# minyoungg/pix2latent

Hardware: AMD Instinct MI355X
Metric: candidate-latent evals/sec (fwd+loss+bwd), BigGAN-256 pop=18 (higher is better)
Workload: dtype f32 (fp32 tensors everywhere; convolutions >= 32x32 and the self-attention multiply on the 16-bit MFMA pipe with fp32-grade operand splits and fp32 accumulate: the 16x16 Winograd, direct and sub-pixel 3x3 kernels and the 1x1 kernels (4x4 layers included) on power-of-two scaled operands in 2 fp16 pie

## Files before the change

pix2latent_amd/csrc/p2l_h2r.hip:

```cpp
#include "p2l_conv_k.h"

#include <atomic>
#include <type_traits>

using namespace p2lconv;

namespace {

#ifndef P2L_H2R_ABL
#define P2L_H2R_ABL 0
#endif

__device__ __forceinline__ int h2c(int c, int row) { return c ^ ((row >> 2) & 3) ^ (((row >> 1) & 1) << 1); }

constexpr int HP = 24, HH = 10, HW = 18;
constexpr int ROWS = HH * HP;
constexpr int PLANE = ROWS * 64 + 32;
constexpr int BUF = 4 * PLANE;
constexpr int EP = 68;
constexpr int DUMP_FLOATS = 4 * 32 * EP;
constexpr int ETAB_FLOATS = 4 * 16 * 12;
constexpr int PTAB_FLOATS = 16 * 8;
constexpr size_t LDS_BYTES = 2 * (size_t)BUF + (DUMP_FLOATS + 32 + ETAB_FLOATS + PTAB_FLOATS) * sizeof(float);

template <int PRO, int EPI>
__global__ __launch_bounds__(256, 1) void conv_h2r_kernel(const ConvK k, const int n_tiles) {
  constexpr bool FAST = EPI != 0, MASK = EPI == 2, POOL = EPI == 3;
  extern __shared__ __attribute__((aligned(16))) float smem[];
  char* As = reinterpret_cast<char*>(smem);
  float* dump = smem + 2 * BUF / 4;
  float* red = dump + DUMP_FLOATS;
  float* etab = red + 32;
  float* ptab = etab + ETAB_FLOATS;

  const int tid = threadIdx.x;
  const int lane = tid & 63, wave = tid >> 6;
  const int l31 = lane & 31, lhi = lane >> 5;
  const int mh = wave >> 1, nt = wave & 1;

  h16x8 bh[36], bm[36];
  {
    const char* wb = reinterpret_cast<const char*>(k.w) + l31 * 64;
    const int oh = h2c(lhi, l31) * 16, om = h2c(2 + lhi, l31) * 16;
#pragma unroll
    for (int s = 0; s < 36; ++s) {
      const int c = s / 9, tap = s - c * 9;
      const char* slab = wb + (size_t)(((c * 2 + nt) * 9 + tap) * 32) * 64;
      bh[s] = *reinterpret_cast<const h16x8*>(slab + oh);
      bm[s] = *reinterpret_cast<const h16x8*>(slab + om);
    }
  }

  const int G = gridDim.x;
  const int v = xcd_remap(blockIdx.x, G);
  const int t_begin = (int)(((long)v * n_tiles) / G), t_end = (int)(((long)(v + 1) * n_tiles) / G);
  const int tiles_per_image = k.tiles_x * k.tiles_y;

  const int cq = tid & 15, p0 = tid >> 4;
  const int goff0 = (-k.W + (p0 - 1)) * k.x_ld + cq * 4;
  const int lplane = (cq >> 2) * PLANE;
  const int loff0 = p0 * 64 + (cq & 1) * 8 + h2c((cq >> 1) & 1, p0) * 16;
  int e_line[2], e_hx[2], e_goff[2], e_loff[2];
#pragma unroll
  for (int e = 0; e < 2; ++e) {
    const int idx = tid + 256 * e;
    e_line[e] = idx < 320 ? (idx >> 5) : -1;
    e_hx[e] = 16 + ((idx >> 4) & 1);
    const int row = (idx >> 5) * HP + e_hx[e];
    e_goff[e] = (((idx >> 5) - 1) * k.W + (e_hx[e] - 1)) * k.x_ld + cq * 4;
    e_loff[e] = row * 64 + (cq & 1) * 8 + h2c((cq >> 1) & 1, row) * 16;
  }
  const int line_step = k.W * k.x_ld;

  int aoff[2][3];
#pragma unroll
  for (int ms = 0; ms < 2; ++ms) {
    const int i = (mh * 2 + ms) * 32 + l31;
    const int Q = i >> 2, s = i & 3;
    const int row0 = (2 * ((Q >> 3) & 3) + (s >> 1)) * HP + 2 * (Q & 7) + (s & 1);
#pragma unroll
    for (int dx = 0; dx < 3; ++dx) aoff[ms][dx] = (row0 + dx) * 64 + h2c(lhi, row0 + dx) * 16;
  }

  float sw, inv_w;
  h2_scales(__builtin_amdgcn_readfirstlane(k.w_tail[0]), sw, inv_w);

  auto image_scales = [&](int b, float& xs, float& os) {
    float a = 0.f, ms_ = 0.f, mt_ = 0.f;
    if (k.amax_in != nullptr) {
      for (int i = tid; i < k.amax_in_n; i += 256) a = fmaxf(a, k.amax_in[(size_t)b * k.amax_in_n + i]);
      if (PRO != P2L_PRO_NONE && !k.amax_in_applied) {
        const f32x4* ps = reinterpret_cast<const f32x4*>(k.pro_s + (size_t)b * k.pro_bstride);
        const f32x4* pt = reinterpret_cast<const f32x4*>(k.pro_t + (size_t)b * k.pro_bstride);
        for (int c = tid; c < (k.Cin >> 2); c += 256) {
          const f32x4 s4 = ps[c], t4 = pt[c];
          ms_ = fmaxf(fmaxf(ms_, fmaxf(fabsf(s4.x), fabsf(s4.y))), fmaxf(fabsf(s4.z), fabsf(s4.w)));
          mt_ = fmaxf(fmaxf(mt_, fmaxf(fabsf(t4.x), fabsf(t4.y))), fmaxf(fabsf(t4.z), fabsf(t4.w)));
        }
      }
    } else if (tid < 64) {
      a = k.amax[b * 64 + tid];
    }
#pragma unroll
    for (int o = 1; o < 64; o <<= 1) {
      a = fmaxf(a, __shfl_xor(a, o, 64));
      if (PRO != P2L_PRO_NONE) { ms_ = fmaxf(ms_, __shfl_xor(ms_, o, 64)); mt_ = fmaxf(mt_, __shfl_xor(mt_, o, 64)); }
    }
    __syncthreads();
    if (lane == 0) { red[wave * 4] = a; red[wave * 4 + 1] = ms_; red[wave * 4 + 2] = mt_; }
    if (PRO != P2L_PRO_NONE && tid < 16) {
      *reinterpret_cast<f32x4*>(ptab + tid * 8) = *reinterpret_cast<const f32x4*>(k.pro_s + (size_t)b * k.pro_bstride + tid * 4);
      *reinterpret_cast<f32x4*>(ptab + tid * 8 + 4) = *reinterpret_cast<const f32x4*>(k.pro_t + (size_t)b * k.pro_bstride + tid * 4);
    }
    __syncthreads();
    a = fmaxf(fmaxf(red[0], red[4]), fmaxf(red[8], red[12]));
    ms_ = fmaxf(fmaxf(red[1], red[5]), fmaxf(red[9], red[13]));
    mt_ = fmaxf(fmaxf(red[2], red[6]), fmaxf(red[10], red[14]));
    if (PRO != P2L_PRO_NONE && k.amax_in != nullptr) a = (k.amax_in_applied ? a : ms_ * a + mt_) * 1.001f;
    float inv_x;
    h2_scales(__builtin_bit_cast(unsigned, a), xs, inv_x);
    os = inv_x * inv_w;
  };

  f32x4 xr[6];
  float st_xs = 1.f;
  char* st_dst = As;
  const float* st_base = k.x;
  bool st_top = false, st_bot = false, st_left = false, st_right = false;
  auto tile_geom = [&](int t, int& b, int& y0, int& x0, int& til) {
    b = t / tiles_per_image;
    til = t - b * tiles_per_image;
    const int ty = til / k.tiles_x;
    y0 = ty << 3; x0 = (til - ty * k.tiles_x) << 4;
  };
  auto item_ok = [&](int it) -> bool {
    if (it < 10) return !((st_top && it == 0) || (st_bot && it == 9) || (st_left && p0 == 0));
    const int e = it - 10;
    return e_line[e] >= 0 && !((st_top && e_line[e] == 0) || (st_bot && e_line[e] == 9) || (st_right && e_hx[e] == 17));
  };
  auto begin_tile = [&](int t, int buf, float xs) {
    int b, y0, x0, til;
    tile_geom(t, b, y0, x0, til);
    st_top = (y0 == 0); st_bot = (y0 + 8 == k.H); st_left = (x0 == 0); st_right = (x0 + 16 == k.W);
    st_xs = xs;
    st_dst = As + buf * BUF;
    st_base = k.x + (size_t)((b * k.H + y0) * k.W + x0) * k.x_ld;
  };
  auto issue = [&](auto half_c) {
    constexpr int half = decltype(half_c)::value;
#pragma unroll
    for (int j = 0; j < 6; ++j) {
      const int it = half * 6 + j;
      const int go = it < 10 ? goff0 + it * line_step : e_goff[it - 10];
      xr[j] = *reinterpret_cast<const f32x4*>(st_base + (item_ok(it) ? go : cq * 4));
    }
  };
  auto land = [&](int it) {
    if (it >= 10 && e_line[it - 10] < 0) return;
    f32x4 v4 = xr[it % 6];
    if (PRO != P2L_PRO_NONE) {
      const f32x4 s4 = *reinterpret_cast<const f32x4*>(ptab + cq * 8), t4 = *reinterpret_cast<const f32x4*>(ptab + cq * 8 + 4);
      v4 = v4 * s4 + t4;
      if (PRO == P2L_PRO_AFFINE_RELU) {
        v4.x = fmaxf(v4.x, 0.f); v4.y = fmaxf(v4.y, 0.f); v4.z = fmaxf(v4.z, 0.f); v4.w = fmaxf(v4.w, 0.f);
      }
    }
    v4 = v4 * (item_ok(it) ? st_xs : 0.f);
    const h16x4 h = __builtin_convertvector(v4, h16x4);
    const f32x4 w = __builtin_convertvector(h, f32x4);
    const h16x4 m = __builtin_convertvector(v4 - w, h16x4);
    const int lo = it < 10 ? ((loff0 + it * (HP * 64)) ^ ((it & 1) ? 32 : 0)) : e_loff[it - 10];
    *reinterpret_cast<h16x4*>(st_dst + lplane + lo) = h;
    *reinterpret_cast<h16x4*>(st_dst + lplane + (lo ^ 32)) = m;
  };
  using Half0 = std::integral_constant<int, 0>;
  using Half1 = std::integral_constant<int, 1>;

  const int e_c4 = lane & 15, e_n = e_c4 * 4;
  float* my_etab = etab + (wave * 16 + e_c4) * 12;
  f32x4 e_bias, e_ns, e_nt;
  if (FAST && lane < 16) {
    *reinterpret_cast<f32x4*>(my_etab) = k.bias ? ld4(k.bias, (unsigned)e_n) : f32x4{0.f, 0.f, 0.f, 0.f};
    *reinterpret_cast<f32x4*>(my_etab + 4) = f32x4{1.f, 1.f, 1.f, 1.f};
    *reinterpret_cast<f32x4*>(my_etab + 8) = f32x4{0.f, 0.f, 0.f, 0.f};
  }
  int e_tab_b = -1;
  const float e_lo = (k.act == P2L_ACT_RELU) ? 0.f : -__builtin_inff();
  int pb = 0, py0 = 0, px0 = 0, ptil = 0;
  float e_amax = 0.f, e_amaxp = 0.f;
  f32x4 ev, ep, em[4];
  unsigned e_pix0 = 0, e_ppix = 0;
  auto epi_tile = [&](int b, int y0_, int x0_, int til_) {
    pb = b; py0 = y0_; px0 = x0_; ptil = til_;
    e_amax = 0.f; e_amaxp = 0.f;
    if (k.amax_ps && b != e_tab_b) {
      if (lane < 16) {
        *reinterpret_cast<f32x4*>(my_etab + 4) = ld4(k.amax_ps, (unsigned)(b * k.amax_pbstride + e_n));
        *reinterpret_cast<f32x4*>(my_etab + 8) = ld4(k.amax_pt, (unsigned)(b * k.amax_pbstride + e_n));
      }
      e_tab_b = b;
    }
  };
  auto epi_addr = [&](int j) {
    const int Q = wave * 8 + j * 4 + (lane >> 4);
    const int oy0 = py0 + 2 * ((Q >> 3) & 3), ox0 = px0 + 2 * (Q & 7);
    e_pix0 = (unsigned)((pb * k.H + oy0) * k.W + ox0);
    e_ppix = (unsigned)((pb * (k.H >> 1) + (oy0 >> 1)) * (k.W >> 1) + (ox0 >> 1));
  };
  auto epi_mask = [&](int j) {
    epi_addr(j);
    if (MASK) {
#pragma unroll
      for (int s = 0; s < 4; ++s)
        em[s] = ld4(k.mask, (e_pix0 + (unsigned)((s >> 1) * k.W + (s & 1))) * (unsigned)k.mask_ld + (unsigned)e_n);
    }
  };
  auto epi_read = [&](int j, int s) {
    ev = *reinterpret_cast<const f32x4*>(dump + wave * 32 * EP + (4 * (j * 4 + (lane >> 4)) + s) * EP + e_c4 * 4);
    if (s == 0) {
      e_bias = *reinterpret_cast<const f32x4*>(my_etab);
      e_ns = *reinterpret_cast<const f32x4*>(my_etab + 4);
      e_nt = *reinterpret_cast<const f32x4*>(my_etab + 8);
    }
  };
  auto epi_px = [&](int s) {
    f32x4 t = ev + e_bias;
    t.x = fmaxf(t.x, e_lo); t.y = fmaxf(t.y, e_lo); t.z = fmaxf(t.z, e_lo); t.w = fmaxf(t.w, e_lo);
    if (MASK) {
      t.x = em[s].x > 0.f ? t.x : 0.f; t.y = em[s].y > 0.f ? t.y : 0.f;
      t.z = em[s].z > 0.f ? t.z : 0.f; t.w = em[s].w > 0.f ? t.w : 0.f;
    }
    st4(k.y, (e_pix0 + (unsigned)((s >> 1) * k.W + (s & 1))) * (unsigned)k.y_ld + (unsigned)e_n, t);
    e_amax = absmax4(e_amax, t * e_ns + e_nt);
    if (POOL) {
      if (s == 0) ep = t;
      else { ep.x = fmaxf(ep.x, t.x); ep.y = fmaxf(ep.y, t.y); ep.z = fmaxf(ep.z, t.z); ep.w = fmaxf(ep.w, t.w); }
    }
  };
  auto epi_pool = [&]() {
    if (POOL) {
      st4(k.yp, e_ppix * (unsigned)k.yp_ld + (unsigned)e_n, ep);
      e_amaxp = absmax4(e_amaxp, ep);
    }
  };
  auto epi_maxima = [&]() {
    if (k.amax_out != nullptr || k.amax_outp != nullptr) {
      float m = e_amax, mp = e_amaxp;
#pragma unroll
      for (int o = 1; o < 64; o <<= 1) { m = fmaxf(m, __shfl_xor(m, o, 64)); mp = fmaxf(mp, __shfl_xor(mp, o, 64)); }
      if (lane == 0) {
        const size_t slot = (size_t)pb * k.amax_out_n + (size_t)ptil * 4 + wave;
        if (k.amax_out != nullptr) k.amax_out[slot] = m;
        if (k.amax_outp != nullptr) k.amax_outp[slot] = mp;
      }
    }
  };
  auto epi_hook = [&](int s) {
    if (s == 0) epi_mask(0);
    if (s >= 5 && s < 9) epi_px(s - 5);
    if (s >= 4 && s < 8) epi_read(0, s - 4);
    if (s == 9) epi_pool();
    if (s == 16) epi_mask(1);
    if (s >= 21 && s < 25) epi_px(s - 21);
    if (s >= 20 && s < 24) epi_read(1, s - 20);
    if (s == 25) epi_pool();
  };

  if (t_begin >= t_end) return;

  int b_cur, y0, x0, til;
  tile_geom(t_begin, b_cur, y0, x0, til);
  float xs_cur, os_cur;
  image_scales(b_cur, xs_cur, os_cur);
  begin_tile(t_begin, 0, xs_cur);
  issue(Half0{});
#pragma unroll
  for (int it = 0; it < 6; ++it) land(it);
  issue(Half1{});
#pragma unroll
  for (int it = 6; it < 12; ++it) land(it);
  __syncthreads();

  auto run_tile = [&](int t, auto with_epi_c) {
    constexpr bool WITH_EPI = decltype(with_epi_c)::value;
    const int cur = (t - t_begin) & 1;
    tile_geom(t, b_cur, y0, x0, til);
    const int tn = (t + 1 < t_end) ? t + 1 : t;
    const int b_next = tn / tiles_per_image;
    float xs_next = xs_cur, os_next = os_cur;
    if (b_next != b_cur) image_scales(b_next, xs_next, os_next);
    begin_tile(tn, cur ^ 1, xs_next);
    if (!(P2L_H2R_ABL & 1)) issue(Half0{});

    const char* Ab = As + cur * BUF;
    f32x16 acc[2];
#pragma unroll
    for (int ms = 0; ms < 2; ++ms)
#pragma unroll
      for (int r = 0; r < 16; ++r) acc[ms][r] = 0.f;

    h16x8 af[2][2][2];
    auto lda = [&](int s, h16x8 (&a)[2][2]) {
      const int c = s / 9, tap = s - c * 9;
      const int dy = tap / 3, dx = tap - dy * 3;
#pragma unroll
      for (int ms = 0; ms < 2; ++ms) {
        const int oh = aoff[ms][dx] ^ ((dy & 1) ? 32 : 0);
        a[ms][0] = *reinterpret_cast<const h16x8*>(Ab + c * PLANE + dy * (HP * 64) + oh);
        a[ms][1] = *reinterpret_cast<const h16x8*>(Ab + c * PLANE + dy * (HP * 64) + (oh ^ 32));
      }
    };
    lda(0, af[0]);
#pragma unroll
    for (int s = 0; s < 36; ++s) {
      if (s + 1 < 36 && !(P2L_H2R_ABL & 16)) lda(s + 1, af[(s + 1) & 1]);
      __builtin_amdgcn_sched_barrier(0);
      const h16x8 (&a)[2][2] = af[s & 1];
      if (!(P2L_H2R_ABL & 2)) {
      acc[0] = __builtin_amdgcn_mfma_f32_32x32x16_f16(a[0][1], bh[s], acc[0], 0, 0, 0);
      acc[1] = __builtin_amdgcn_mfma_f32_32x32x16_f16(a[1][1], bh[s], acc[1], 0, 0, 0);
      acc[0] = __builtin_amdgcn_mfma_f32_32x32x16_f16(a[0][0], bm[s], acc[0], 0, 0, 0);
      acc[1] = __builtin_amdgcn_mfma_f32_32x32x16_f16(a[1][0], bm[s], acc[1], 0, 0, 0);
      acc[0] = __builtin_amdgcn_mfma_f32_32x32x16_f16(a[0][0], bh[s], acc[0], 0, 0, 0);
      acc[1] = __builtin_amdgcn_mfma_f32_32x32x16_f16(a[1][0], bh[s], acc[1], 0, 0, 0);
      } else { acc[0][s & 15] += (float)a[0][0][0] * (float)bh[s][0] + (float)a[1][1][1] * (float)bm[s][1]; }
      if (!(P2L_H2R_ABL & 1)) {
        if (s >= 10 && s < 16) land(s - 10);
        if (s == 15) issue(Half1{});
        if (s >= 28 && s < 34) land(s - 28 + 6);
      }
      if (WITH_EPI && !(P2L_H2R_ABL & 32)) epi_hook(s);
      __builtin_amdgcn_sched_barrier(0);
    }
    if (WITH_EPI) epi_maxima();

#pragma unroll
    for (int ms = 0; ms < 2; ++ms)
#pragma unroll
      for (int r = 0; r < 16; ++r) acc[ms][r] *= os_cur;
    __syncthreads();
    if (!(P2L_H2R_ABL & 8) || acc[0][0] == 12345.678f)
#pragma unroll
    for (int ms = 0; ms < 2; ++ms) {
      float* tb = dump + (mh * 2 + ms) * 32 * EP + nt * 32 + l31;
#pragma unroll
      for (int r = 0; r < 16; ++r) tb[((r & 3) + 8 * (r >> 2) + 4 * lhi) * EP] = acc[ms][r];
    }
    __syncthreads();
    if (FAST) {
      epi_tile(b_cur, y0, x0, til);
    } else {
      if (!(P2L_H2R_ABL & 4) || acc[0][0] == 12345.678f)
      epilogue_vec_items<2>(k, dump, wave, lane, b_cur, y0, x0, 0, til, 0, 0, 0);
    }
    xs_cur = xs_next; os_cur = os_next;
  };
  if (FAST) {
    run_tile(t_begin, std::false_type{});
    for (int t = t_begin + 1; t < t_end; ++t) run_tile(t, std::true_type{});
#pragma unroll
    for (int s = 0; s < 36; ++s) epi_hook(s);
    epi_maxima();
  } else {
    for (int t = t_begin; t < t_end; ++t) run_tile(t, std::false_type{});
  }
}

}

bool p2l_h2r_shape(int taps, int ups, int H, int W, int Cin, int Cout, int x_ld) {
#ifdef P2L_AB_NO_H2R
  return false;
#endif
  return taps == 9 && ups == 0 && Cin == 64 && Cout == 64 && H % 8 == 0 && W % 16 == 0 && x_ld % 4 == 0;
}

static int h2r_epi(const ConvK& k) {
  if (!k.arb_x && !k.res && !k.oscale && !k.noise && k.alpha == 1.0f && k.y != nullptr && k.n_store == 64 &&
      (k.act == P2L_ACT_NONE || k.act == P2L_ACT_RELU) && !(k.form & P2L_FORM_H2R_SEQ_EPI)) {
    if (k.pool == P2L_POOL_NONE) return k.mask ? 2 : 1;
    if (k.pool == P2L_POOL_MAX && !k.mask && k.yp != nullptr) return 3;
  }
  return 0;
}
bool p2l_h2r_takes(const ConvK& k) { return h2r_epi(k) != 0 || (k.form & P2L_FORM_H2R_SEQ_EPI); }

int p2l_h2r_launch(const ConvK& k_in, int pro, hipStream_t st) {
  ConvK k = k_in;
  k.n_ntiles = 1;
  const int n_tiles = k.B * k.tiles_x * k.tiles_y;
  static std::atomic<int> n_cu{0};
  if (n_cu == 0) {
    int dev = 0, cus = 0;
    (void)hipGetDevice(&dev);
    if (hipDeviceGetAttribute(&cus, hipDeviceAttributeMultiprocessorCount, dev) != hipSuccess || cus < 1) cus = 256;
    n_cu = cus;
  }
  const int grid = n_tiles < n_cu ? n_tiles : (int)n_cu;
  const int epi = h2r_epi(k);
#define P2L_H2RL(PROV)                                                                        \
  do {                                                                                        \
    if (epi == 1) P2L_H2RE(PROV, 1); else if (epi == 2) P2L_H2RE(PROV, 2);                    \
    else if (epi == 3) P2L_H2RE(PROV, 3); else P2L_H2RE(PROV, 0);                             \
  } while (0)
#define P2L_H2RE(PROV, EPIV)                                                                  \
  do {                                                                                        \
    auto kfn = conv_h2r_kernel<PROV, EPIV>;                                                   \
    static std::atomic<bool> attr_set{false};                                                 \
    if (!attr_set) {                                                                          \
      (void)hipFuncSetAttribute((const void*)kfn, hipFuncAttributeMaxDynamicSharedMemorySize, \
                                160 * 1024);                                                  \
      attr_set = true;                                                                        \
    }                                                                                         \
    hipLaunchKernelGGL(kfn, dim3(grid), dim3(256), LDS_BYTES, st, k, n_tiles);                \
  } while (0)
  if (pro == P2L_PRO_NONE) P2L_H2RL(P2L_PRO_NONE);
  else if (pro == P2L_PRO_AFFINE_RELU) P2L_H2RL(P2L_PRO_AFFINE_RELU);
  else P2L_H2RL(P2L_PRO_AFFINE);
#undef P2L_H2RL
#undef P2L_H2RE
  return p2l_check_launch();
}
```

Baseline: 1214.

## Add fused arbitrary-gradient epilogue to h2r conv and stream weights via ring

Adds a new EPI==4 path to the 64x64 3x3 half-split conv kernel that fuses a backward-style affine/ReLU-mask gradient epilogue: it masks the conv output by the sign of the recomputed pre-activation, scales it, stores it, and reduces the per-channel sums of g*x and g into per-block partials. That lets these layers use the fast persistent kernel instead of the generic path. The fused paths also stream the last NR weight slices through a small register ring loaded a few steps ahead instead of holding all 36 slices in registers, which lowers register pressure at the cost of extra in-loop loads. Also adds 32-bit offset-fit checks and per-device caching of CU count and attributes.

```diff
diff --git a/pix2latent_amd/csrc/p2l_h2r.hip b/pix2latent_amd/csrc/p2l_h2r.hip
--- a/pix2latent_amd/csrc/p2l_h2r.hip
+++ b/pix2latent_amd/csrc/p2l_h2r.hip
@@ -21,35 +21,48 @@
 constexpr int DUMP_FLOATS = 4 * 32 * EP;
 constexpr int ETAB_FLOATS = 4 * 16 * 12;
 constexpr int PTAB_FLOATS = 16 * 8;
-constexpr size_t LDS_BYTES = 2 * (size_t)BUF + (DUMP_FLOATS + 32 + ETAB_FLOATS + PTAB_FLOATS) * sizeof(float);
+constexpr int ARED_FLOATS = 2 * 4 * 64;
+constexpr size_t LDS_BYTES = 2 * (size_t)BUF + (DUMP_FLOATS + 32 + ETAB_FLOATS + PTAB_FLOATS + ARED_FLOATS) * sizeof(float);
+static_assert(LDS_BYTES <= 160 * 1024, "one block per CU: the whole LDS and no more");
+
+constexpr int RB_AHEAD = 3, RB_SLOTS = RB_AHEAD + 1;
+#ifndef P2L_H2R_NR_FWD
+#define P2L_H2R_NR_FWD 8
+#endif
+#ifndef P2L_H2R_NR_ARB
+#define P2L_H2R_NR_ARB 24
+#endif
 
 template <int PRO, int EPI>
 __global__ __launch_bounds__(256, 1) void conv_h2r_kernel(const ConvK k, const int n_tiles) {
-  constexpr bool FAST = EPI != 0, MASK = EPI == 2, POOL = EPI == 3;
+  constexpr bool FAST = EPI != 0, MASK = EPI == 2, POOL = EPI == 3, ARB = EPI == 4;
   extern __shared__ __attribute__((aligned(16))) float smem[];
   char* As = reinterpret_cast<char*>(smem);
   float* dump = smem + 2 * BUF / 4;
   float* red = dump + DUMP_FLOATS;
   float* etab = red + 32;
   float* ptab = etab + ETAB_FLOATS;
+  float* ared = ptab + PTAB_FLOATS;
 
   const int tid = threadIdx.x;
   const int lane = tid & 63, wave = tid >> 6;
   const int l31 = lane & 31, lhi = lane >> 5;
   const int mh = wave >> 1, nt = wave & 1;
 
-  h16x8 bh[36], bm[36];
-  {
-    const char* wb = reinterpret_cast<const char*>(k.w) + l31 * 64;
-    const int oh = h2c(lhi, l31) * 16, om = h2c(2 + lhi, l31) * 16;
-#pragma unroll
-    for (int s = 0; s < 36; ++s) {
-      const int c = s / 9, tap = s - c * 9;
-      const char* slab = wb + (size_t)(((c * 2 + nt) * 9 + tap) * 32) * 64;
-      bh[s] = *reinterpret_cast<const h16x8*>(slab + oh);
-      bm[s] = *reinterpret_cast<const h16x8*>(slab + om);
-    }
-  }
+  constexpr int NR = EPI == 4 ? P2L_H2R_NR_ARB : EPI != 0 ? P2L_H2R_NR_FWD : 0;
+  constexpr int R0 = 36 - NR;
+  static_assert(NR == 0 || R0 >= RB_AHEAD, "the ring is filled inside the stream");
+  h16x8 bh[36], bm[36], rbh[RB_SLOTS], rbm[RB_SLOTS];
+  const unsigned w_oh = (unsigned)(nt * 9 * 2048 + l31 * 64 + h2c(lhi, l31) * 16);
+  const unsigned w_om = (unsigned)(nt * 9 * 2048 + l31 * 64 + h2c(2 + lhi, l31) * 16);
+  auto ldw = [&](int s, h16x8& h, h16x8& m) {
+    const int c = s / 9, tap = s - c * 9;
+    const char* slab = reinterpret_cast<const char*>(k.w) + (c * 18 + tap) * 2048;
+    h = *reinterpret_cast<const h16x8*>(slab + w_oh);
+    m = *reinterpret_cast<const h16x8*>(slab + w_om);
+  };
+#pragma unroll
+  for (int s = 0; s < R0; ++s) ldw(s, bh[s], bm[s]);
 
   const int G = gridDim.x;
   const int v = xcd_remap(blockIdx.x, G);
@@ -179,7 +192,7 @@
   const int e_c4 = lane & 15, e_n = e_c4 * 4;
   float* my_etab = etab + (wave * 16 + e_c4) * 12;
   f32x4 e_bias, e_ns, e_nt;
-  if (FAST && lane < 16) {
+  if (FAST && !ARB && lane < 16) {
     *reinterpret_cast<f32x4*>(my_etab) = k.bias ? ld4(k.bias, (unsigned)e_n) : f32x4{0.f, 0.f, 0.f, 0.f};
     *reinterpret_cast<f32x4*>(my_etab + 4) = f32x4{1.f, 1.f, 1.f, 1.f};
     *reinterpret_cast<f32x4*>(my_etab + 8) = f32x4{0.f, 0.f, 0.f, 0.f};
@@ -189,11 +202,23 @@
   int pb = 0, py0 = 0, px0 = 0, ptil = 0;
   float e_amax = 0.f, e_amaxp = 0.f;
   f32x4 ev, ep, em[4];
+  f32x4 a_sgx[2], a_sg[2];
+  const bool a_nomask = k.arb_nomask != 0;
   unsigned e_pix0 = 0, e_ppix = 0;
   auto epi_tile = [&](int b, int y0_, int x0_, int til_) {
     pb = b; py0 = y0_; px0 = x0_; ptil = til_;
     e_amax = 0.f; e_amaxp = 0.f;
-    if (k.amax_ps && b != e_tab_b) {
+    if (ARB) {
+#pragma unroll
+      for (int j = 0; j < 2; ++j) { a_sgx[j] = f32x4{0.f, 0.f, 0.f, 0.f}; a_sg[j] = f32x4{0.f, 0.f, 0.f, 0.f}; }
+      if (b != e_tab_b) {
+        if (lane < 16) {
+          *reinterpret_cast<f32x4*>(my_etab) = ld4(k.arb_s, (unsigned)(b * k.arb_bstride + e_n));
+          *reinterpret_cast<f32x4*>(my_etab + 4) = ld4(k.arb_t, (unsigned)(b * k.arb_bstride + e_n));
+        }
+        e_tab_b = b;
+      }
+    } else if (k.amax_ps && b != e_tab_b) {
       if (lane < 16) {
         *reinterpret_cast<f32x4*>(my_etab + 4) = ld4(k.amax_ps, (unsigned)(b * k.amax_pbstride + e_n));
         *reinterpret_cast<f32x4*>(my_etab + 8) = ld4(k.amax_pt, (unsigned)(b * k.amax_pbstride + e_n));
@@ -214,16 +239,34 @@
       for (int s = 0; s < 4; ++s)
         em[s] = ld4(k.mask, (e_pix0 + (unsigned)((s >> 1) * k.W + (s & 1))) * (unsigned)k.mask_ld + (unsigned)e_n);
     }
+    if (ARB) {
+#pragma unroll
+      for (int s = 0; s < 4; ++s)
+        em[s] = ld4(k.arb_x, (e_pix0 + (unsigned)((s >> 1) * k.W + (s & 1))) * (unsigned)k.arb_x_ld + (unsigned)e_n);
+    }
   };
   auto epi_read = [&](int j, int s) {
     ev = *reinterpret_cast<const f32x4*>(dump + wave * 32 * EP + (4 * (j * 4 + (lane >> 4)) + s) * EP + e_c4 * 4);
     if (s == 0) {
       e_bias = *reinterpret_cast<const f32x4*>(my_etab);
       e_ns = *reinterpret_cast<const f32x4*>(my_etab + 4);
-      e_nt = *reinterpret_cast<const f32x4*>(my_etab + 8);
-    }
-  };
-  auto epi_px = [&](int s) {
+      if (!ARB) e_nt = *reinterpret_cast<const f32x4*>(my_etab + 8);
+    }
+  };
+  auto epi_px = [&](int j, int s) {
+    if (ARB) {
+      const f32x4 xv = em[s];
+      const f32x4 pre = xv * e_bias + e_ns;
+      f32x4 g = ev;
+      g.x = (a_nomask || pre.x > 0.f) ? g.x : 0.f; g.y = (a_nomask || pre.y > 0.f) ? g.y : 0.f;
+      g.z = (a_nomask || pre.z > 0.f) ? g.z : 0.f; g.w = (a_nomask || pre.w > 0.f) ? g.w : 0.f;
+      const f32x4 o = g * e_bias;
+      st4(k.y, (e_pix0 + (unsigned)((s >> 1) * k.W + (s & 1))) * (unsigned)k.y_ld + (unsigned)e_n, o);
+      e_amax = absmax4(e_amax, o);
+      a_sgx[j] += g * xv;
+      a_sg[j] += g;
+      return;
+    }
     f32x4 t = ev + e_bias;
     t.x = fmaxf(t.x, e_lo); t.y = fmaxf(t.y, e_lo); t.z = fmaxf(t.z, e_lo); t.w = fmaxf(t.w, e_lo);
     if (MASK) {
@@ -255,13 +298,41 @@
       }
     }
   };
+  auto epi_arb_wave = [&]() {
+    f32x4 sgx = a_sgx[0], sg = a_sg[0], sgx2 = a_sgx[1], sg2 = a_sg[1];
+#pragma unroll
+    for (int o = 16; o < 64; o <<= 1) {
+      sgx.x += __shfl_xor(sgx.x, o, 64); sgx.y += __shfl_xor(sgx.y, o, 64);
+      sgx.z += __shfl_xor(sgx.z, o, 64); sgx.w += __shfl_xor(sgx.w, o, 64);
+      sg.x += __shfl_xor(sg.x, o, 64); sg.y += __shfl_xor(sg.y, o, 64);
+      sg.z += __shfl_xor(sg.z, o, 64); sg.w += __shfl_xor(sg.w, o, 64);
+      sgx2.x += __shfl_xor(sgx2.x, o, 64); sgx2.y += __shfl_xor(sgx2.y, o, 64);
+      sgx2.z += __shfl_xor(sgx2.z, o, 64); sgx2.w += __shfl_xor(sgx2.w, o, 64);
+      sg2.x += __shfl_xor(sg2.x, o, 64); sg2.y += __shfl_xor(sg2.y, o, 64);
+      sg2.z += __shfl_xor(sg2.z, o, 64); sg2.w += __shfl_xor(sg2.w, o, 64);
+    }
+    sgx = sgx + sgx2; sg = sg + sg2;
+    if (lane < 16) {
+      *reinterpret_cast<f32x4*>(ared + wave * 64 + lane * 4) = sgx;
+      *reinterpret_cast<f32x4*>(ared + (4 + wave) * 64 + lane * 4) = sg;
+    }
+  };
+  auto epi_arb_block = [&]() {
+    if (tid < 64) {
+      const float a = (ared[tid] + ared[64 + tid]) + (ared[128 + tid] + ared[192 + tid]);
+      const float t = (ared[256 + tid] + ared[320 + tid]) + (ared[384 + tid] + ared[448 + tid]);
+      const size_t o = ((size_t)pb * k.arb_nblk + ptil) * k.Cout + tid;
+      k.arb_partial[o] = a;
+      k.arb_partial[(size_t)k.B * k.arb_nblk * k.Cout + o] = t;
+    }
+  };
   auto epi_hook = [&](int s) {
     if (s == 0) epi_mask(0);
-    if (s >= 5 && s < 9) epi_px(s - 5);
+    if (s >= 5 && s < 9) epi_px(0, s - 5);
     if (s >= 4 && s < 8) epi_read(0, s - 4);
     if (s == 9) epi_pool();
     if (s == 16) epi_mask(1);
-    if (s >= 21 && s < 25) epi_px(s - 21);
+    if (s >= 21 && s < 25) epi_px(1, s - 21);
     if (s >= 20 && s < 24) epi_read(1, s - 20);
     if (s == 25) epi_pool();
   };
@@ -316,14 +387,18 @@
       if (s + 1 < 36 && !(P2L_H2R_ABL & 16)) lda(s + 1, af[(s + 1) & 1]);
       __builtin_amdgcn_sched_barrier(0);
       const h16x8 (&a)[2][2] = af[s & 1];
+      if (NR != 0 && s + RB_AHEAD >= R0 && s + RB_AHEAD < 36)
+        ldw(s + RB_AHEAD, rbh[(s + RB_AHEAD) % RB_SLOTS], rbm[(s + RB_AHEAD) % RB_SLOTS]);
+      const h16x8& b_h = s < R0 ? bh[s] : rbh[s % RB_SLOTS];
+      const h16x8& b_m = s < R0 ? bm[s] : rbm[s % RB_SLOTS];
       if (!(P2L_H2R_ABL & 2)) {
-      acc[0] = __builtin_amdgcn_mfma_f32_32x32x16_f16(a[0][1], bh[s], acc[0], 0, 0, 0);
-      acc[1] = __builtin_amdgcn_mfma_f32_32x32x16_f16(a[1][1], bh[s], acc[1], 0, 0, 0);
-      acc[0] = __builtin_amdgcn_mfma_f32_32x32x16_f16(a[0][0], bm[s], acc[0], 0, 0, 0);
-      acc[1] = __builtin_amdgcn_mfma_f32_32x32x16_f16(a[1][0], bm[s], acc[1], 0, 0, 0);
-      acc[0] = __builtin_amdgcn_mfma_f32_32x32x16_f16(a[0][0], bh[s], acc[0], 0, 0, 0);
-      acc[1] = __builtin_amdgcn_mfma_f32_32x32x16_f16(a[1][0], bh[s], acc[1], 0, 0, 0);
-      } else { acc[0][s & 15] += (float)a[0][0][0] * (float)bh[s][0] + (float)a[1][1][1] * (float)bm[s][1]; }
+      acc[0] = __builtin_amdgcn_mfma_f32_32x32x16_f16(a[0][1], b_h, acc[0], 0, 0, 0);
+      acc[1] = __builtin_amdgcn_mfma_f32_32x32x16_f16(a[1][1], b_h, acc[1], 0, 0, 0);
+      acc[0] = __builtin_amdgcn_mfma_f32_32x32x16_f16(a[0][0], b_m, acc[0], 0, 0, 0);
+      acc[1] = __builtin_amdgcn_mfma_f32_32x32x16_f16(a[1][0], b_m, acc[1], 0, 0, 0);
+      acc[0] = __builtin_amdgcn_mfma_f32_32x32x16_f16(a[0][0], b_h, acc[0], 0, 0, 0);
+      acc[1] = __builtin_amdgcn_mfma_f32_32x32x16_f16(a[1][0], b_h, acc[1], 0, 0, 0);
+      } else { acc[0][s & 15] += (float)a[0][0][0] * (float)b_h[0] + (float)a[1][1][1] * (float)b_m[1]; }
       if (!(P2L_H2R_ABL & 1)) {
         if (s >= 10 && s < 16) land(s - 10);
         if (s == 15) issue(Half1{});
@@ -333,12 +408,14 @@
       __builtin_amdgcn_sched_barrier(0);
     }
     if (WITH_EPI) epi_maxima();
+    if (WITH_EPI && ARB) epi_arb_wave();
 
 #pragma unroll
     for (int ms = 0; ms < 2; ++ms)
 #pragma unroll
       for (int r = 0; r < 16; ++r) acc[ms][r] *= os_cur;
     __syncthreads();
+    if (WITH_EPI && ARB) epi_arb_block();
     if (!(P2L_H2R_ABL & 8) || acc[0][0] == 12345.678f)
 #pragma unroll
     for (int ms = 0; ms < 2; ++ms) {
@@ -361,6 +438,11 @@
 #pragma unroll
     for (int s = 0; s < 36; ++s) epi_hook(s);
     epi_maxima();
+    if (ARB) {
+      epi_arb_wave();
+      __syncthreads();
+      epi_arb_block();
+    }
   } else {
     for (int t = t_begin; t < t_end; ++t) run_tile(t, std::false_type{});
   }
@@ -375,29 +457,56 @@
   return taps == 9 && ups == 0 && Cin == 64 && Cout == 64 && H % 8 == 0 && W % 16 == 0 && x_ld % 4 == 0;
 }
 
+extern "C" int p2l_h2r_offsets_fit(long long B, long long H, long long W, long long ld) {
+  return B > 0 && H > 0 && W > 0 && ld > 0 && B * H * W <= ((1ll << 32) - 1) / ld;
+}
+static bool h2r_fits(const ConvK& k) {
+  int ld = k.x_ld;
+  if (k.y && k.y_ld > ld) ld = k.y_ld;
+  if (k.yp && k.yp_ld > ld) ld = k.yp_ld;
+  if (k.res && k.res_ld > ld) ld = k.res_ld;
+  if (k.mask && k.mask_ld > ld) ld = k.mask_ld;
+  if (k.arb_x && k.arb_x_ld > ld) ld = k.arb_x_ld;
+  if (k.arb_skip && k.arb_skip_ld > ld) ld = k.arb_skip_ld;
+  return p2l_h2r_offsets_fit(k.B, k.H, k.W, ld) != 0;
+}
+
 static int h2r_epi(const ConvK& k) {
-  if (!k.arb_x && !k.res && !k.oscale && !k.noise && k.alpha == 1.0f && k.y != nullptr && k.n_store == 64 &&
-      (k.act == P2L_ACT_NONE || k.act == P2L_ACT_RELU) && !(k.form & P2L_FORM_H2R_SEQ_EPI)) {
+  if (k.res || k.oscale || k.noise || k.alpha != 1.0f || k.y == nullptr || k.n_store != 64 ||
+      (k.form & P2L_FORM_H2R_SEQ_EPI))
+    return 0;
+  if (k.arb_x)
+    return (k.pool == P2L_POOL_NONE && !k.arb_skip && !k.mask && !k.bias && k.act == P2L_ACT_NONE && !k.pro_s &&
+            !k.pro_t && k.arb_s && k.arb_t && k.arb_partial && k.amax_out) ? 4 : 0;
+  if (k.act == P2L_ACT_NONE || k.act == P2L_ACT_RELU) {
     if (k.pool == P2L_POOL_NONE) return k.mask ? 2 : 1;
     if (k.pool == P2L_POOL_MAX && !k.mask && k.yp != nullptr) return 3;
   }
   return 0;
 }
-bool p2l_h2r_takes(const ConvK& k) { return h2r_epi(k) != 0 || (k.form & P2L_FORM_H2R_SEQ_EPI); }
+bool p2l_h2r_takes(const ConvK& k) {
+  return h2r_fits(k) && (h2r_epi(k) != 0 || (k.form & P2L_FORM_H2R_SEQ_EPI));
+}
 
 int p2l_h2r_launch(const ConvK& k_in, int pro, hipStream_t st) {
   ConvK k = k_in;
   k.n_ntiles = 1;
   const int n_tiles = k.B * k.tiles_x * k.tiles_y;
-  static std::atomic<int> n_cu{0};
+  constexpr int MAXDEV = 64;
+  int dev = 0;
+  if (hipGetDevice(&dev) != hipSuccess) return P2L_ELAUNCH;
+  const bool cached = dev >= 0 && dev < MAXDEV;
+  static std::atomic<int> n_cu_dev[MAXDEV];
+  int n_cu = cached ? n_cu_dev[dev].load() : 0;
   if (n_cu == 0) {
-    int dev = 0, cus = 0;
-    (void)hipGetDevice(&dev);
+    int cus = 0;
     if (hipDeviceGetAttribute(&cus, hipDeviceAttributeMultiprocessorCount, dev) != hipSuccess || cus < 1) cus = 256;
     n_cu = cus;
+    if (cached) n_cu_dev[dev] = cus;
   }
-  const int grid = n_tiles < n_cu ? n_tiles : (int)n_cu;
+  const int grid = n_tiles < n_cu ? n_tiles : n_cu;
   const int epi = h2r_epi(k);
+  if (epi == 4 && pro != P2L_PRO_NONE) return P2L_EUNSUP;
 #define P2L_H2RL(PROV)                                                                        \
   do {                                                                                        \
     if (epi == 1) P2L_H2RE(PROV, 1); else if (epi == 2) P2L_H2RE(PROV, 2);                    \
@@ -406,15 +515,16 @@
 #define P2L_H2RE(PROV, EPIV)                                                                  \
   do {                                                                                        \
     auto kfn = conv_h2r_kernel<PROV, EPIV>;                                                   \
-    static std::atomic<bool> attr_set{false};                                                 \
-    if (!attr_set) {                                                                          \
-      (void)hipFuncSetAttribute((const void*)kfn, hipFuncAttributeMaxDynamicSharedMemorySize, \
-                                160 * 1024);                                                  \
-      attr_set = true;                                                                        \
+    static std::atomic<bool> attr_set[MAXDEV];                                                \
+    if (!cached || !attr_set[dev]) {                                                          \
+      if (hipFuncSetAttribute((const void*)kfn, hipFuncAttributeMaxDynamicSharedMemorySize,   \
+                              160 * 1024) != hipSuccess) return P2L_ELAUNCH;                     \
+      if (cached) attr_set[dev] = true;                                                       \
     }                                                                                         \
     hipLaunchKernelGGL(kfn, dim3(grid), dim3(256), LDS_BYTES, st, k, n_tiles);                \
   } while (0)
-  if (pro == P2L_PRO_NONE) P2L_H2RL(P2L_PRO_NONE);
+  if (epi == 4) P2L_H2RE(P2L_PRO_NONE, 4);
+  else if (pro == P2L_PRO_NONE) P2L_H2RL(P2L_PRO_NONE);
   else if (pro == P2L_PRO_AFFINE_RELU) P2L_H2RL(P2L_PRO_AFFINE_RELU);
   else P2L_H2RL(P2L_PRO_AFFINE);
 #undef P2L_H2RL
```

Result: no change. 1219 (median of 6 runs) (+0.4%).
